# optimato/UMPA

Hardware: AMD Instinct MI355X
Metric: Mpixels/s (output map) at Nw=5, max_shift=5, 10 frames (higher is better)
Workload: dtype f64; 1 GPU; C2: 2048x2048, 10 frames, Nw=5, max_shift=5, dark-field on; output_pixels_per_gpu=4112784, parallelism=1 GPU

## Files before the change

umpa_amd/csrc/umpa_tiled.h:

```cpp
#pragma once
#include "umpa_direct.h"
#include "umpa_corr.h"
#include "umpa_march.h"
#include "umpa_masked.h"
#include <mutex>
#include <vector>
#include <functional>

namespace umpa {

struct Maps {
    double* SamSq;
    double* RefSq;
    double* WS;
    double* MR;
    int H, W;
    int br0, br1, bc0, bc1, Wf;
};

typedef double map_pair_t __attribute__((ext_vector_type(2)));
__host__ __device__ __forceinline__ size_t map_at(int k, size_t x, size_t plane) { return ((size_t)(k >> 1) * plane + x) * 2 + (k & 1); }

template <int NW>
struct PrepCfg {
    static constexpr int T = UMPA_TILE, S = 2 * NW + 1, Q = T + 2 * NW, QP = Q | 1, NT = 256, CB = 8;
    static constexpr int RAW = Q * QP;
    static constexpr int HPL = T * QP;
    static constexpr size_t LDS = (size_t)(RAW + 2 * HPL) * sizeof(double);
};

template <int KIND, int NW>
__global__ void __launch_bounds__(256, NW <= 5 ? 3 : 2)
prep_maps_kernel(ModelDev m, Maps M, Sep1D sep, int ntx, int nty, int sides, int tx0, int ty0)
{
    const bool do_ref = (sides & 2) != 0;
    using C = PrepCfg<NW>;
    extern __shared__ __attribute__((aligned(16))) char smem_raw[];
    double* raw = reinterpret_cast<double*>(smem_raw);
    double* hpl = raw + C::RAW;

    const int lin = xcd_band_remap(blockIdx.x, ntx * nty);
    if (lin >= ntx * nty) return;
    const int tx = tx0 + lin % ntx, ty = ty0 + lin / ntx;
    const int r0 = NW + ty * C::T, c0 = NW + tx * C::T;
    const int tid = threadIdx.x;
    const size_t plane = (size_t)M.H * M.W;

    const int vc = tid & 31, vrb = (tid >> 5) & 3, vsq = tid >> 7;
    double acc[2][C::CB];
#pragma unroll
    for (int o = 0; o < C::CB; o++) acc[0][o] = acc[1][o] = 0.0;

    constexpr int NS = (C::Q * C::Q + C::NT - 1) / C::NT;
    int s_lds[NS], s_g[NS];
    {
#pragma unroll
        for (int n = 0; n < NS; n++) {
            const int it = tid + n * C::NT, c = it % C::Q, r = it / C::Q;
            s_lds[n] = it < C::Q * C::Q ? c * C::QP + r : -1;
            s_g[n] = min(max(r0 - NW + r, M.br0), M.br1) * M.Wf + min(max(c0 - NW + c, M.bc0), M.bc1);
        }
    }
    double pp[NS];
    auto fetch = [&](int k, int st) {
        const FrameDesc f = load_frame(m.frames, k);
        const long shift = (long)f.pi * M.Wf + f.pj;
        const UMPA_GLOBAL double* src = gp(st ? f.ref : f.sam);
#pragma unroll
        for (int n = 0; n < NS; n++) pp[n] = src[s_g[n] - shift];
    };
    fetch(0, 0);
    for (int k = 0; k < m.Na; k++) {
#pragma unroll
        for (int st = 0; st < 2; st++) {
            if (st == 1 && !do_ref) break;
            __syncthreads();
#pragma unroll
            for (int n = 0; n < NS; n++)
                if (s_lds[n] >= 0) raw[s_lds[n]] = pp[n];
            if (st == 0 && do_ref) fetch(k, 1);
            else if (k + 1 < m.Na) fetch(k + 1, 0);
            __syncthreads();
            if (tid < 4 * C::Q) {
                const int r = tid % C::Q, cb = tid / C::Q;
                const double* src = raw + (cb * C::CB) * C::QP + r;
                double lin_[C::CB], sq_[C::CB];
#pragma unroll
                for (int o = 0; o < C::CB; o++) { lin_[o] = 0.0; sq_[o] = 0.0; }
#pragma unroll
                for (int t = 0; t < C::CB + C::S - 1; t++) {
                    const double v = src[t * C::QP];
                    const double v2 = v * v;
#pragma unroll
                    for (int o = 0; o < C::CB; o++) {
                        const int tap = t - o;
                        if (tap >= 0 && tap < C::S) { lin_[o] = fma(sep.hc[tap], v, lin_[o]); sq_[o] = fma(sep.hc[tap], v2, sq_[o]); }
                    }
                }
                double* dl = hpl + (cb * C::CB) * C::QP + r;
                double* dq = dl + C::HPL;
#pragma unroll
                for (int o = 0; o < C::CB; o++) { dl[o * C::QP] = lin_[o]; dq[o * C::QP] = sq_[o]; }
            }
            __syncthreads();
            if (!(KIND == 0 && vsq == 0)) {
                double out[C::CB];
                fir_block<NW, C::CB>(hpl + vsq * C::HPL + vc * C::QP + vrb * C::CB, 1, sep.hr, out);
                const int gc = c0 + vc;
                const bool odd = (k & 1) != 0, last = k + 1 == m.Na;
                UMPA_GLOBAL double* dstmap = gpw(st == 0 ? M.WS : M.MR);
#pragma unroll
                for (int o = 0; o < C::CB; o++) {
                    const int gr = r0 + vrb * C::CB + o;
                    const bool inside = gr < M.H - NW && gc < M.W - NW;
                    if (vsq == 1) acc[st][o] += out[o];
                    else {
                        const double v = st == 0 ? out[o] : out[o] / m.win_sum;
                        if (odd) {
                            if (inside) {
                                map_pair_t pv; pv[0] = acc[st][o]; pv[1] = v;
                                *reinterpret_cast<UMPA_GLOBAL map_pair_t*>(dstmap + map_at(k - 1, (size_t)gr * M.W + gc, plane)) = pv;
                            }
                        } else if (last) {
                            if (inside) dstmap[map_at(k, (size_t)gr * M.W + gc, plane)] = v;
                        } else acc[st][o] = v;
                    }
                }
            }
        }
    }
    const int gc = c0 + vc;
#pragma unroll
    for (int o = 0; o < C::CB; o++) {
        const int gr = r0 + vrb * C::CB + o;
        if (gr >= M.H - NW || gc >= M.W - NW) continue;
        const size_t g = (size_t)gr * M.W + gc;
        if (vsq == 1) {
            gpw(M.SamSq)[g] = acc[0][o];
            if (do_ref) gpw(M.RefSq)[g] = acc[1][o];
        }
    }
}

struct ReplayArgs {
    const double* table;
    size_t slot_stride;
    int drow0, N1d;
    int strip_w, tw, drows;
    int row0, rows;
    int bw_log2;
    int ablate;
};

#define UMPA_KFIX 16
#define UMPA_KTEMPL 24

__device__ __forceinline__ double ld_off(const UMPA_GLOBAL double* base, unsigned byte_off)
{
    return *reinterpret_cast<const UMPA_GLOBAL double*>(reinterpret_cast<const UMPA_GLOBAL char*>(base) + byte_off);
}
__device__ __forceinline__ map_pair_t ld_pair_off(const UMPA_GLOBAL double* base, unsigned byte_off)
{
    return *reinterpret_cast<const UMPA_GLOBAL map_pair_t*>(reinterpret_cast<const UMPA_GLOBAL char*>(base) + byte_off);
}

struct PixConst { double t1, t3, t2, t6; };


__device__ __forceinline__ unsigned table_slot(int ms, int si, int sj) { const int UJ = 2 * ms - 1; return (unsigned)((si + ms - 1) * UJ + (sj + ms - 1)); }
__device__ __forceinline__ size_t sample_at(int W, int ref_mode, int i, int j, int si, int sj) { return ref_mode ? (size_t)(i - si) * W + (j - sj) : (size_t)i * W + j; }
__device__ __forceinline__ size_t reference_at(int W, int ref_mode, int i, int j, int si, int sj) { return ref_mode ? (size_t)i * W + j : (size_t)(i + si) * W + (j + sj); }

template <int KIND, int NA>
__device__ __forceinline__ int eval_lookup(const ModelDev& m, const Maps& M, const ReplayArgs& R, int ref_mode,
                                           int i, int j, size_t tpx, int si, int sj,
                                           const double* fixed, const PixConst& pc, double& cost, Fit& fit)
{
    const int ms = m.ms;
    if (si <= -ms || si >= ms) return UMPA_ST_BOUND;
    if (sj <= -ms) return UMPA_ST_BOUND | UMPA_ST_DIM;
    if (sj >= ms) return UMPA_ST_BOUND | UMPA_ST_DIM | UMPA_ST_POSITIVE;
    const double t5 = gp(R.table)[(size_t)table_slot(ms, si, sj) * (unsigned)R.slot_stride + tpx];
    const size_t xs = sample_at(M.W, ref_mode, i, j, si, sj), xr = reference_at(M.W, ref_mode, i, j, si, sj);
    const double rwt = 1.0 / (double)m.Nwt;
    double t1 = pc.t1, t3 = pc.t3;
    if (ref_mode) t1 = NA > 0 ? ld_off(gp(M.SamSq), (unsigned)xs * 8u) : gp(M.SamSq)[xs];
    else t3 = NA > 0 ? ld_off(gp(M.RefSq), (unsigned)xr * 8u) : gp(M.RefSq)[xr];
    if (KIND == 1) {
        double t2 = 0.0, t4 = 0.0;
        const size_t plane = (size_t)M.H * M.W;
        if (NA > 0) {
            const unsigned bm = (unsigned)(ref_mode ? xs : xr) * 16u;
            const UMPA_GLOBAL double* __restrict__ mov = gp(ref_mode ? M.WS : M.MR);
            map_pair_t mp[NA > 0 ? (NA + 1) / 2 : 1];
#pragma unroll
            for (int q = 0; q < (NA + 1) / 2; q++) mp[q] = ld_pair_off(mov + (size_t)q * 2 * plane, bm);
#pragma unroll
            for (int k = 0; k < NA; k++) { const double a = mp[k >> 1][k & 1]; t4 = fma(a, fixed[k], t4); t2 = fma(a, a, t2); }
        } else {
            const UMPA_GLOBAL double* __restrict__ mov = gp(ref_mode ? M.WS : M.MR);
            const size_t xm = ref_mode ? xs : xr;
            double mv[UMPA_KFIX];
#pragma unroll
            for (int k = 0; k < UMPA_KFIX; k++) mv[k] = k < m.Na ? mov[map_at(k, xm, plane)] : 0.0;
#pragma unroll
            for (int k = 0; k < UMPA_KFIX; k++) if (k < m.Na) { t4 = fma(mv[k], fixed[k], t4); t2 = fma(mv[k], mv[k], t2); }
            if (m.Na > UMPA_KFIX) {
                const UMPA_GLOBAL double* __restrict__ fx = gp(ref_mode ? M.MR : M.WS);
                const size_t xf = ref_mode ? xr : xs;
                for (int k = UMPA_KFIX; k < m.Na; k++) { const double a = mov[map_at(k, xm, plane)]; t4 = fma(a, fx[map_at(k, xf, plane)], t4); t2 = fma(a, a, t2); }
            }
        }
        double t6;
        if (ref_mode) { t2 = pc.t2; t6 = pc.t6; }
        else t6 = m.win_sum * t2;
        solve_rcp<KIND>(t1, t2, t3, t4, t5, t6, rwt, cost, fit);
    } else solve_rcp<KIND>(t1, 0.0, t3, 0.0, t5, 0.0, rwt, cost, fit);
    return UMPA_ST_OK;
}

template <int NA>
struct LookupRaw {
    double t5, sq;
    map_pair_t mp[NA > 0 ? (NA + 1) / 2 : 1];
};

template <int KIND, int NA>
__device__ __forceinline__ void lookup_load(const ModelDev& m, const Maps& M, const ReplayArgs& R, int ref_mode,
                                            int i, int j, size_t tpx, int si, int sj, LookupRaw<NA>& raw)
{
    raw.t5 = gp(R.table)[(size_t)table_slot(m.ms, si, sj) * (unsigned)R.slot_stride + tpx];
    const size_t xs = sample_at(M.W, ref_mode, i, j, si, sj), xr = reference_at(M.W, ref_mode, i, j, si, sj);
    raw.sq = ref_mode ? ld_off(gp(M.SamSq), (unsigned)xs * 8u) : ld_off(gp(M.RefSq), (unsigned)xr * 8u);
    if (KIND == 1) {
        const size_t plane = (size_t)M.H * M.W;
        const unsigned bm = (unsigned)(ref_mode ? xs : xr) * 16u;
        const UMPA_GLOBAL double* __restrict__ mov = gp(ref_mode ? M.WS : M.MR);
#pragma unroll
        for (int q = 0; q < (NA + 1) / 2; q++) raw.mp[q] = ld_pair_off(mov + (size_t)q * 2 * plane, bm);
    }
}

template <int KIND, int NA>
__device__ __forceinline__ void lookup_solve(const ModelDev& m, int ref_mode, const LookupRaw<NA>& raw,
                                             const double* fixed, const PixConst& pc, double& cost, Fit& fit)
{
    const double rwt = 1.0 / (double)m.Nwt;
    double t1 = pc.t1, t3 = pc.t3, t6 = 0.0, t2 = 0.0, t4 = 0.0;
    if (ref_mode) t1 = raw.sq; else t3 = raw.sq;
    if (KIND == 1) {
#pragma unroll
        for (int k = 0; k < NA; k++) { const double a = raw.mp[k >> 1][k & 1]; t4 = fma(a, fixed[k], t4); t2 = fma(a, a, t2); }
        if (ref_mode) { t2 = pc.t2; t6 = pc.t6; }
        else t6 = m.win_sum * t2;
    }
    solve_rcp<KIND>(t1, t2, t3, t4, raw.t5, t6, rwt, cost, fit);
}

#ifndef UMPA_REPLAY_ROWS
#define UMPA_REPLAY_ROWS 1
#endif
#define UMPA_REPLAY_THREADS (64 * UMPA_REPLAY_ROWS)
#ifndef UMPA_REPLAY_SPECULATE
#define UMPA_REPLAY_SPECULATE 1
#endif
#define UMPA_REPLAY_SPECULATE_NA 11

template <int KIND, int NA, bool OD>
__global__ void __launch_bounds__(UMPA_REPLAY_THREADS, 3)
replay_walk_kernel(ModelDev m, Maps M, ReplayArgs R, RegionArgs A, OdArgs od_in)
{
    OdArgs od = od_in;
    if (!OD) od.mode = 0;
    __shared__ double memo_lds[25 * UMPA_REPLAY_THREADS];
    const LdsMemo<UMPA_REPLAY_THREADS> memo = {memo_lds + threadIdx.y * 64 + threadIdx.x};
    const int nparked = od.mode == 3 ? __builtin_amdgcn_readfirstlane(gp(od.cnt_in)[OD_C_PX]) : 0;
  for (int q = (blockIdx.y * gridDim.x + blockIdx.x) * UMPA_REPLAY_THREADS + threadIdx.y * 64 + threadIdx.x, first = 1;;
       q += gridDim.x * gridDim.y * UMPA_REPLAY_THREADS, first = 0) {
    int xi, xj;
    bool live;
    if (od.mode == 3) {
        if (__builtin_amdgcn_readfirstlane(q & ~63) >= nparked) break;
        live = q < nparked;
        const int pxq = live ? gp(od.px_in)[q] : 0;
        xi = pxq / A.N1; xj = pxq - xi * A.N1;
    } else if (od.mode == 1) {
        if (!first) break;
        live = od_seed_pixel(od, R.drow0, A.step0, A.step1, xi, xj);
        live = live && xi >= R.row0 && xi < R.row0 + R.rows && xj < A.N1;
    } else {
        if (!first) break;
        if (OD && od.sub > 1) {
            xj = (blockIdx.x * 64 + threadIdx.x) * od.sub + (od.sub >> 1);
            xi = (blockIdx.y * UMPA_REPLAY_ROWS + threadIdx.y) * od.sub + (od.sub >> 1);
        } else {
            const int bwl = R.bw_log2;
            xj = (blockIdx.x << bwl) + (threadIdx.x & ((1 << bwl) - 1));
            xi = ((blockIdx.y * UMPA_REPLAY_ROWS + threadIdx.y) << (6 - bwl)) + (threadIdx.x >> bwl);
        }
        xi += R.row0;
        live = xi < R.row0 + R.rows && xj < A.N1;
    }
    const size_t px = (size_t)xi * A.pitch + xj;
    size_t tpx = (size_t)(xi * A.step0 - R.drow0) * R.N1d + (size_t)xj * A.step1;
    if (R.strip_w > 0) {
        const int dc = xj * A.step1, strip = dc / R.strip_w, UJr = 2 * m.ms - 1;
        tpx = (((size_t)strip * R.drows + (size_t)(xi * A.step0 - R.drow0)) * (size_t)(UJr * UJr)) * R.tw + (size_t)(dc - strip * R.strip_w);
    }
    if (live && A.cover && gp(A.cover)[px] < A.thr) live = false;
    OdLane L;
    if (live && !od_begin(od, xi * A.step0 - R.drow0, xj * A.step1, L)) live = false;
    if (live) {
    const int i = A.org0 + A.step0 * xi, j = A.org1 + A.step1 * xj;
    constexpr int NFIX = NA > 0 ? NA : UMPA_KFIX;
    double fixed[NFIX];
    if (KIND == 1) {
        const size_t plane = (size_t)M.H * M.W, x0 = (size_t)i * M.W + j;
        const UMPA_GLOBAL double* __restrict__ fx = gp(m.ref_mode ? M.MR : M.WS);
        if constexpr (NA > 0) {
#pragma unroll
            for (int qq = 0; qq < (NA + 1) / 2; qq++) {
                const map_pair_t v = *reinterpret_cast<const UMPA_GLOBAL map_pair_t*>(fx + ((size_t)qq * plane + x0) * 2);
                fixed[2 * qq] = v[0];
                if (2 * qq + 1 < NFIX) fixed[2 * qq + 1] = v[1];
            }
        } else {
#pragma unroll
            for (int k = 0; k < NFIX; k++) fixed[k] = k < m.Na ? fx[map_at(k, x0, plane)] : 0.0;
        }
    }
    PixConst pc = {0.0, 0.0, 0.0, 0.0};
    {
        const size_t x0 = (size_t)i * M.W + j;
        if (m.ref_mode) {
            pc.t3 = gp(M.RefSq)[x0];
            if (KIND == 1) {
#pragma unroll
                for (int k = 0; k < NFIX; k++) if (NA > 0 || k < m.Na) pc.t2 = fma(fixed[k], fixed[k], pc.t2);
                for (int k = NFIX; k < m.Na; k++) { const double a = gp(M.MR)[map_at(k, x0, (size_t)M.H * M.W)]; pc.t2 = fma(a, a, pc.t2); }
                pc.t6 = m.win_sum * pc.t2;
            }
        } else pc.t1 = gp(M.SamSq)[x0];
    }
    Walk w;
    walk_begin(w, memo, A.uv ? gp(A.uv)[2 * px] : 0.0, A.uv ? gp(A.uv)[2 * px + 1] : 0.0);
    if (R.ablate & 1) {
        double csum = 0.0;
        Fit fit = w.live;
        for (int n = 0; n < 18; n++) {
            double c = 0.0;
            eval_lookup<KIND, NA>(m, M, R, m.ref_mode, i, j, tpx, (n % 5) - 2, (n / 5) - 2, fixed, pc, c, fit);
            csum += c;
        }
        w.out = csum; w.live = fit; w.phase = PH_DONE; w.status = 1;
    }
    const int sigma = m.ref_mode ? -1 : 1;
    while (w.phase < PH_FIT) {
        if (!od_check(od, L, m.ms, sigma, w.req_i, w.req_j)) break;
        double c = 0.0;
        Fit fit = w.live;
        if constexpr (!OD && NA > 0 && NA <= UMPA_REPLAY_SPECULATE_NA && UMPA_REPLAY_SPECULATE) {
            int si = w.req_i, sj = w.req_j;
            const bool spec = walk_speculate(w, si, sj);
            const int st = shift_status(m.ms, w.req_i, w.req_j), st2 = shift_status(m.ms, si, sj);
            const bool ok1 = st == UMPA_ST_OK, ok2 = st2 == UMPA_ST_OK;
            LookupRaw<NA> r1, r2;
            lookup_load<KIND, NA>(m, M, R, m.ref_mode, i, j, tpx, ok1 ? w.req_i : 0, ok1 ? w.req_j : 0, r1);
            lookup_load<KIND, NA>(m, M, R, m.ref_mode, i, j, tpx, ok2 ? si : 0, ok2 ? sj : 0, r2);
            double c2 = 0.0;
            Fit fit2 = w.live;
            lookup_solve<KIND, NA>(m, m.ref_mode, r1, fixed, pc, c, fit);
            lookup_solve<KIND, NA>(m, m.ref_mode, r2, fixed, pc, c2, fit2);
            walk_feed(w, memo, st, c, fit, m.call_cap);
            if (spec && w.phase < PH_FIT && w.req_i == si && w.req_j == sj) walk_feed(w, memo, st2, c2, fit2, m.call_cap);
        } else {
            const int st = eval_lookup<KIND, NA>(m, M, R, m.ref_mode, i, j, tpx, w.req_i, w.req_j, fixed, pc, c, fit);
            walk_feed(w, memo, st, c, fit, m.call_cap);
        }
    }
    if (L.miss) od_park(od, L, xi * A.N1 + xj);
    else if (!(OD && od.sub > 1)) {
        double nb[16];
        walk_finish(w, memo, (R.ablate & 2) ? 0 : m.subpx, nb);
        if (KIND == 1 && (w.live.t != 0.0 || w.live.v != 0.0))
            w.live.v = w.live.v / w.live.t;
        store_pixel(A, px, KIND, w, memo, nb);
    }
    }
    if (od.mode == 1) od_record_visited(od, L, live);
  }
}

typedef hipError_t (*TableConsumer)(void* user, const ModelDev& dev, const Maps& M, const ReplayArgs& R, const RegionArgs& A,
                                    hipStream_t s);

struct TiledState {
    TableConsumer consumer = nullptr;  void* consumer_user = nullptr;
    double* maps = nullptr;   size_t maps_cap = 0;
    double* table = nullptr;  size_t table_cap = 0;
    bool table_limited = false;
    Sep1D sep;
    bool separable = false;
    int sep_nw = -1;
    bool ref_maps_ok = false;
    int ref_kind = -1, ref_K = 0;
    size_t ref_plane = 0;
    int ref_rect[4] = {0, 0, 0, 0};
    void* od_buf = nullptr;   size_t od_cap = 0;
    int* od_host = nullptr;   int od_slot = 0;
    const int* stat_slots[64];  int stat_n = 0;
    double stat_total_passes = 0.0;
};
#define UMPA_OD_SLOTS 256

struct TimedLaunch { int name; hipEvent_t t0, t1; double fma; const int* counts; double fma_per; };

struct TiledTimers {
    std::vector<TimedLaunch>* out;
    std::function<hipEvent_t()> get;
    hipStream_t s;
    size_t first;
    bool open = false;
    TiledTimers(std::vector<TimedLaunch>* out_, std::function<hipEvent_t()> get_, hipStream_t s_)
        : out(out_), get(std::move(get_)), s(s_), first(out_ ? out_->size() : 0) {}
    void tic(int name)
    {
        open = false;
        if (!out) return;
        TimedLaunch en = {name, get(), get(), 0.0, nullptr, 0.0};
        if (!en.t0 || !en.t1) return;
        (void)hipEventRecord(en.t0, s);
// ... 891 lines not shown
```

Baseline: 1649 Mpx/s.

## Stream interior prep tiles via double-buffered LDS DMA and row-major horizontal filter

```diff
diff --git a/umpa_amd/csrc/umpa_tiled.h b/umpa_amd/csrc/umpa_tiled.h
--- a/umpa_amd/csrc/umpa_tiled.h
+++ b/umpa_amd/csrc/umpa_tiled.h
@@ -24,9 +24,12 @@
 template <int NW>
 struct PrepCfg {
     static constexpr int T = UMPA_TILE, S = 2 * NW + 1, Q = T + 2 * NW, QP = Q | 1, NT = 256, CB = 8;
-    static constexpr int RAW = Q * QP;
+    static constexpr int P = (Q / 2) | 1, NDMA = 128, NPIECE = Q * P, NPT = (NPIECE + NDMA - 1) / NDMA;
+    static constexpr int RAW = NPT * NDMA * 2;
     static constexpr int HPL = T * QP;
-    static constexpr size_t LDS = (size_t)(RAW + 2 * HPL) * sizeof(double);
+    static constexpr size_t LDS = (size_t)(2 * RAW + 2 * HPL) * sizeof(double);
+    static constexpr int HNB = NT / Q, HB = ((T + HNB - 1) / HNB + 1) & ~1, HNU = (T + HB - 1) / HB;
+    static constexpr int HIN = (HB + S - 1) / 2;
 };
 
 template <int KIND, int NW>
@@ -37,7 +40,7 @@
     using C = PrepCfg<NW>;
     extern __shared__ __attribute__((aligned(16))) char smem_raw[];
     double* raw = reinterpret_cast<double*>(smem_raw);
-    double* hpl = raw + C::RAW;
+    double* hpl = raw + 2 * C::RAW;
 
     const int lin = xcd_band_remap(blockIdx.x, ntx * nty);
     if (lin >= ntx * nty) return;
@@ -51,29 +54,118 @@
 #pragma unroll
     for (int o = 0; o < C::CB; o++) acc[0][o] = acc[1][o] = 0.0;
 
-    constexpr int NS = (C::Q * C::Q + C::NT - 1) / C::NT;
-    int s_lds[NS], s_g[NS];
-    {
+    const int hr_ = tid % C::Q, hcb = tid / C::Q;
+    const int hc0 = min(hcb * C::HB, C::T - C::HB), hdup = hcb * C::HB - hc0;
+    auto h_stage = [&](const double* slot) {
+        if (tid < C::HNU * C::Q) {
+            const map_pair_t* src = reinterpret_cast<const map_pair_t*>(slot) + hr_ * C::P + hc0 / 2;
+            map_pair_t in[C::HIN];
+#pragma unroll
+            for (int j = 0; j < C::HIN; j++) in[j] = src[j];
+            double lin_[C::HB], sq_[C::HB];
+#pragma unroll
+            for (int o = 0; o < C::HB; o++) { lin_[o] = 0.0; sq_[o] = 0.0; }
+#pragma unroll
+            for (int t = 0; t < C::HB + C::S - 1; t++) {
+                const double v = in[t >> 1][t & 1];
+                const double v2 = v * v;
+#pragma unroll
+                for (int o = 0; o < C::HB; o++) {
+                    const int tap = t - o;
+                    if (tap >= 0 && tap < C::S) { lin_[o] = fma(sep.hc[tap], v, lin_[o]); sq_[o] = fma(sep.hc[tap], v2, sq_[o]); }
+                }
+            }
+            double* dl = hpl + hc0 * C::QP + hr_;
+            double* dq = dl + C::HPL;
+#pragma unroll
+            for (int o = 0; o < C::HB; o++)
+                if (o >= hdup) { dl[o * C::QP] = lin_[o]; dq[o * C::QP] = sq_[o]; }
+        }
+    };
+    auto v_stage = [&](int k, auto ST) {
+        constexpr int st = decltype(ST)::value;
+        if (!(KIND == 0 && vsq == 0)) {
+            double out[C::CB];
+            fir_block<NW, C::CB>(hpl + vsq * C::HPL + vc * C::QP + vrb * C::CB, 1, sep.hr, out);
+            const int gc = c0 + vc;
+            const bool odd = (k & 1) != 0, last = k + 1 == m.Na;
+            UMPA_GLOBAL double* dstmap = gpw(st == 0 ? M.WS : M.MR);
+#pragma unroll
+            for (int o = 0; o < C::CB; o++) {
+                const int gr = r0 + vrb * C::CB + o;
+                const bool inside = gr < M.H - NW && gc < M.W - NW;
+                if (vsq == 1) acc[st][o] += out[o];
+                else {
+                    const double v = st == 0 ? out[o] : out[o] / m.win_sum;
+                    if (odd) {
+                        if (inside) {
+                            map_pair_t pv; pv[0] = acc[st][o]; pv[1] = v;
+                            *reinterpret_cast<UMPA_GLOBAL map_pair_t*>(dstmap + map_at(k - 1, (size_t)gr * M.W + gc, plane)) = pv;
+                        }
+                    } else if (last) {
+                        if (inside) dstmap[map_at(k, (size_t)gr * M.W + gc, plane)] = v;
+                    } else acc[st][o] = v;
+                }
+            }
+        }
+    };
+    using Sam = std::integral_constant<int, 0>;
+    using Ref = std::integral_constant<int, 1>;
+
+    const bool interior = r0 - NW >= M.br0 && r0 - NW + C::Q - 1 <= M.br1 && c0 - NW >= M.bc0 && c0 - NW + C::Q - 1 <= M.bc1;
+    if (interior) {
+        const int np = do_ref ? 2 * m.Na : m.Na;
+        const bool dma_wave = tid >= C::NT - C::NDMA;
+        const int w = max(tid - (C::NT - C::NDMA), 0);
+        const unsigned wave_piece0 = (unsigned)__builtin_amdgcn_readfirstlane(w & ~63);
+        unsigned src_off[C::NPT];
+#pragma unroll
+        for (int i = 0; i < C::NPT; i++) {
+            const int p = w + i * C::NDMA, r = min(p / C::P, C::Q - 1), c2 = min(p % C::P, C::Q / 2 - 1);
+            src_off[i] = (unsigned)((r0 - NW + r) * M.Wf + (c0 - NW + 2 * c2)) * 8u;
+        }
+        auto issue = [&](int n) {
+            const FrameDesc f = load_frame(m.frames, do_ref ? n >> 1 : n);
+            const long shift = ((long)f.pi * M.Wf + f.pj) * 8;
+            const UMPA_GLOBAL char* g = (const UMPA_GLOBAL char*)gp((do_ref && (n & 1)) ? f.ref : f.sam) - shift;
+            UMPA_LDS_AS char* slot = (UMPA_LDS_AS char*)(raw + (n & 1) * C::RAW);
+#pragma unroll
+            for (int i = 0; i < C::NPT; i++) lds_dma16(g, src_off[i], slot + (size_t)(wave_piece0 + i * C::NDMA) * 16);
+        };
+        int n = 0;
+        auto round = [&](int k, auto ST) {
+            if (dma_wave) { if (n + 1 < np) wait_vmcnt<C::NPT>(); else wait_vmcnt<0>(); }
+            lds_barrier();
+            h_stage(raw + (n & 1) * C::RAW);
+            lds_barrier();
+            if (dma_wave && n + 2 < np) issue(n + 2);
+            v_stage(k, ST);
+            n++;
+        };
+        if (dma_wave) { issue(0); if (np > 1) issue(1); }
+        for (int k = 0; k < m.Na; k++) {
+            round(k, Sam{});
+            if (do_ref) round(k, Ref{});
+        }
+    } else {
+        constexpr int NS = (C::Q * C::Q + C::NT - 1) / C::NT;
+        int s_lds[NS], s_g[NS];
 #pragma unroll
         for (int n = 0; n < NS; n++) {
             const int it = tid + n * C::NT, c = it % C::Q, r = it / C::Q;
-            s_lds[n] = it < C::Q * C::Q ? c * C::QP + r : -1;
+            s_lds[n] = it < C::Q * C::Q ? r * (2 * C::P) + c : -1;
             s_g[n] = min(max(r0 - NW + r, M.br0), M.br1) * M.Wf + min(max(c0 - NW + c, M.bc0), M.bc1);
         }
-    }
-    double pp[NS];
-    auto fetch = [&](int k, int st) {
-        const FrameDesc f = load_frame(m.frames, k);
-        const long shift = (long)f.pi * M.Wf + f.pj;
-        const UMPA_GLOBAL double* src = gp(st ? f.ref : f.sam);
-#pragma unroll
-        for (int n = 0; n < NS; n++) pp[n] = src[s_g[n] - shift];
-    };
-    fetch(0, 0);
-    for (int k = 0; k < m.Na; k++) {
-#pragma unroll
-        for (int st = 0; st < 2; st++) {
-            if (st == 1 && !do_ref) break;
+        double pp[NS];
+        auto fetch = [&](int k, int st) {
+            const FrameDesc f = load_frame(m.frames, k);
+            const long shift = (long)f.pi * M.Wf + f.pj;
+            const UMPA_GLOBAL double* src = gp(st ? f.ref : f.sam);
+#pragma unroll
+            for (int n = 0; n < NS; n++) pp[n] = src[s_g[n] - shift];
+        };
+        auto round = [&](int k, auto ST) {
+            constexpr int st = decltype(ST)::value;
             __syncthreads();
 #pragma unroll
             for (int n = 0; n < NS; n++)
@@ -81,52 +173,14 @@
             if (st == 0 && do_ref) fetch(k, 1);
             else if (k + 1 < m.Na) fetch(k + 1, 0);
             __syncthreads();
-            if (tid < 4 * C::Q) {
-                const int r = tid % C::Q, cb = tid / C::Q;
-                const double* src = raw + (cb * C::CB) * C::QP + r;
-                double lin_[C::CB], sq_[C::CB];
-#pragma unroll
-                for (int o = 0; o < C::CB; o++) { lin_[o] = 0.0; sq_[o] = 0.0; }
-#pragma unroll
-                for (int t = 0; t < C::CB + C::S - 1; t++) {
-                    const double v = src[t * C::QP];
-                    const double v2 = v * v;
-#pragma unroll
-                    for (int o = 0; o < C::CB; o++) {
-                        const int tap = t - o;
-                        if (tap >= 0 && tap < C::S) { lin_[o] = fma(sep.hc[tap], v, lin_[o]); sq_[o] = fma(sep.hc[tap], v2, sq_[o]); }
-                    }
-                }
-                double* dl = hpl + (cb * C::CB) * C::QP + r;
-                double* dq = dl + C::HPL;
-#pragma unroll
-                for (int o = 0; o < C::CB; o++) { dl[o * C::QP] = lin_[o]; dq[o * C::QP] = sq_[o]; }
-            }
+            h_stage(raw);
             __syncthreads();
-            if (!(KIND == 0 && vsq == 0)) {
-                double out[C::CB];
-                fir_block<NW, C::CB>(hpl + vsq * C::HPL + vc * C::QP + vrb * C::CB, 1, sep.hr, out);
-                const int gc = c0 + vc;
-                const bool odd = (k & 1) != 0, last = k + 1 == m.Na;
-                UMPA_GLOBAL double* dstmap = gpw(st == 0 ? M.WS : M.MR);
-#pragma unroll
-                for (int o = 0; o < C::CB; o++) {
-                    const int gr = r0 + vrb * C::CB + o;
-                    const bool inside = gr < M.H - NW && gc < M.W - NW;
-                    if (vsq == 1) acc[st][o] += out[o];
-                    else {
-                        const double v = st == 0 ? out[o] : out[o] / m.win_sum;
-                        if (odd) {
-                            if (inside) {
-                                map_pair_t pv; pv[0] = acc[st][o]; pv[1] = v;
-                                *reinterpret_cast<UMPA_GLOBAL map_pair_t*>(dstmap + map_at(k - 1, (size_t)gr * M.W + gc, plane)) = pv;
-                            }
-                        } else if (last) {
-                            if (inside) dstmap[map_at(k, (size_t)gr * M.W + gc, plane)] = v;
-                        } else acc[st][o] = v;
-                    }
-                }
-            }
+            v_stage(k, ST);
+        };
+        fetch(0, 0);
+        for (int k = 0; k < m.Na; k++) {
+            round(k, Sam{});
+            if (do_ref) round(k, Ref{});
         }
     }
     const int gc = c0 + vc;
```

Result: no change. 1650 Mpx/s, median of 4 (+0.1%).
